# thanosDelatolas/eva-vos

Measured on AMD Instinct MI355X. Metric: frames/sec STCN mask-propagate 480p 1-obj, higher is better.
Workload: dtype f32; 1 GPU; DAVIS-17-val-shaped 480x854 (padded 480x864) single-object STCN propagate: fresh engine, interact(mask,0), T=66 frames/video, mem_freq=5, top_k=50; one video per step per GPU; videos_per_gpu=38, streams_per_gpu=4, key_lookahead=0, clips=8 distinct synthetic clips (one per pooled engine), weights=synthetic recipe seed 0 (no checkpoints offline)

## Files before the change

eva_vos_amd/_lib.py:

```python
from __future__ import annotations

import ctypes as C
import os

import torch

_HERE = os.path.dirname(os.path.abspath(__file__))
LIB_PATH = os.environ.get("STCN_LIB") or os.path.join(_HERE, "libstcn_hip.so")

K_CLASSES = ("conv", "conv_reduce", "memread", "elementwise", "conv_n1", "other", "wino_input", "fusion_conv", "attention")


class WeightDesc(C.Structure):
    _fields_ = [("name", C.c_char_p), ("data", C.c_void_p), ("ndim", C.c_int32), ("shape", C.c_int64 * 4)]


class EngineOpts(C.Structure):
    _fields_ = [(n, C.c_int32) for n in ("lookahead", "decode_batch", "key_batch", "fuse_side")]


class ModelOpts(C.Structure):
    _fields_ = [("top_k", C.c_int32), ("km", C.c_float)]


# ... 22 lines not shown
    "stcn_test_transpose": (_I, [_P, _P, _P, _I, _I, _I, _L, _L, _I]),
    "stcn_engine_create": (_I, [_P, _I, _I, _I, _I, _I, _P, _P, _P, _P, C.POINTER(_P)]),
    "stcn_engine_create_ex": (_I, [_P, _I, _I, _I, _I, _I, _P, _P, _P, _P, C.POINTER(EngineOpts), C.POINTER(_P)]),
    "stcn_engine_get_opts": (_I, [_P, C.POINTER(EngineOpts)]),
    "stcn_engine_destroy": (_I, [_P]),
    "stcn_engine_reset": (_I, [_P]),
    "stcn_engine_clone": (_I, [_P, _P, _P, _P, C.POINTER(_P)]),
    "stcn_interact": (_I, [_P, _P, _I, _I, _I]),
    "stcn_get_stats": (_I, [_P, C.POINTER(Stats)]),
    "stcn_get_flops": (_I, [_P, C.POINTER(_D)]),
    "stcn_last_conv_path": (C.c_char_p, []),
    "stcn_test_conv_trace": (_I, [_I]),
    "stcn_test_conv_trace_get": (C.c_char_p, []),
    "stcn_test_conv": (_I, [_P, _P, _P, _P, _P, _P] + [_I] * 11),
    "stcn_test_conv_ex": (_I, [_P, _P, _P, _P, _P, _P] + [_I] * 11 + [_P, _I, _L, _L, _L, _I, _L]),
    "stcn_test_conv_path": (_I, [_I] * 9 + [C.c_char_p, _I]),
    "stcn_test_conv_plan": (_I, [_I] * 9 + [C.POINTER(C.c_int32), _I, C.POINTER(_D)]),
    "stcn_test_sweep_plan": (_I, [_I, _I, _I, _I, C.POINTER(C.c_int32), _I, C.POINTER(C.c_int32)]),
    "stcn_test_encode_key": (_I, [_P, _P, _P, _I, _I, _P, _P, _P, _P, _P]),
    "stcn_test_encode_value": (_I, [_P, _P, _P, _P, _P, _I, _I, _I, _P]),
    "stcn_test_memory_read": (_I, [_P, _P, _P, _P, _I, _I, _I, _P, _P, _P]),
    "stcn_test_memory_read_k": (_I, [_P, _P, _P, _P, _I, _I, _I, _I, _P, _P, _P]),
    "stcn_test_memory_read_km": (_I, [_P, _P, _P, _P, _I, _I, _I, _I, _I, _I, _F, _P, _P, _P, _P]),
    "stcn_bench_memory_read": (_I, [_P, _P, _P, _P, _I, _I, _I, _I, _P, C.POINTER(_F), C.POINTER(C.c_int32)]),
    "stcn_bench_memory_read_k": (_I, [_P, _P, _P, _P, _I, _I, _I, _I, _I, _P, C.POINTER(_F), C.POINTER(C.c_int32)]),
    "stcn_bench_memory_read_km": (_I, [_P, _P, _P, _P, _I, _I, _I, _I, _I, _I, _F, _I, _P, C.POINTER(_F), C.POINTER(C.c_int32)]),
    "stcn_memread_plan": (_I, [_I, _I, C.POINTER(C.c_int32)]),
    "stcn_memread_scratch": (_I, [_I, C.POINTER(C.c_int64)]),
    "stcn_test_kernel": (_I, [C.c_char_p, _P, C.POINTER(_P), _I, C.POINTER(C.c_int64), _I, C.POINTER(_D), _I]),
    "stcn_test_fail_at": (_I, [_I]),
# ... 63 lines not shown
```

eva_vos_amd/csrc/engine.cpp:

```cpp
#include "engine.h"
#include "src_hash.h"

#include <algorithm>
#include <atomic>
#include <cmath>
#include <cstdarg>
#include <cstdio>
#include <cstdlib>
#include <cstring>
#include <map>
#include <mutex>
#include <unordered_map>
#include <utility>

namespace stcn {

static thread_local char g_err[512] = "";
void set_error(const char *fmt, ...) {
    va_list ap;
    va_start(ap, fmt);
    vsnprintf(g_err, sizeof(g_err), fmt, ap);
    va_end(ap);
}
const char *get_error() { return g_err; }
// ... 480 lines not shown
    p.kn = w.kn;
    pl = ConvPlan{};
    pl.fl = 2.0 * p.M * p.N * (double)(cw.kh * cw.kw * cw.cin);
    if (a.force_splitk <= 0 && (fusion_conv_plan(p, pl) || wino4_plan(p, m.wino4_min_wg, w.wino_v_floats, w.splitk_floats, pl) ||
                                wino_plan(p, w.wino_v_floats, w.splitk_floats, pl)))
        return STCN_OK;
    conv_plan(p, a.force_splitk, w.splitk_floats, pl);
    return STCN_OK;
}

int run_conv(const Model &m, Work &w, hipStream_t s, const std::string &name, const ConvArgs &a) {
    ConvP p;
    ConvPlan &pl = g_path.plan;
    const int rc = plan_conv(m, w, name, a, p, pl);
    if (rc) return rc;
    hipEvent_t *eg[W4_MAX_CHUNKS] = {}, *ei[W4_MAX_CHUNKS] = {}, *er = nullptr;
    if (w.prof) {
        const double in0 = (double)(p.bs0 ? p.B : 1) * p.H * p.W * p.c0, in1 = p.x1 ? (double)(p.bs1 ? p.B : 1) * p.H * p.W * p.c1 : 0.0;
        const double resb = p.res ? (p.res_bs ? (double)p.M * p.N : (double)p.OH * p.OW * p.N) : 0.0;
        const double bytes = 4.0 * (in0 + in1 + (double)p.N * p.K + (double)p.M * p.N + resb);
        const bool hbm_bound = pl.fl / bytes < 157.3e12 / 8.0e12;
        const int cls = w.conv_cls;
        const bool hbm_acc = hbm_bound && cls == STCN_K_CONV;
        w.prof->bytes[cls] += bytes;
        w.prof->flops[cls] += pl.fl;
        w.prof->exec_flops[cls] += pl.fl_exec;
        if (hbm_acc) { w.prof->hbm_conv_bytes += bytes; w.prof->hbm_conv_flops += pl.fl; }
        if (pl.family == CONV_WINO4) w.prof->wino4_flops += pl.fl; else if (pl.family == CONV_WINO2) w.prof->wino2_flops += pl.fl;
        for (int c = 0; c < pl.n_gemm; ++c) {
            eg[c] = w.prof->attach(cls, hbm_acc);
            if (c < pl.n_in) ei[c] = w.prof->attach(STCN_K_WINO_INPUT);
        }
        if (pl.reduce) er = w.prof->attach(STCN_K_CONV_REDUCE);
    }
    if (g_trace_on) { char b[96]; g_trace += name; g_trace += '='; g_trace += format_conv_path(pl, b, sizeof(b)); g_trace += '\n'; }
    switch (pl.family) {
    case CONV_FUSION: fusion_conv_launch(p, pl, s, eg[0]); break;
    case CONV_WINO4: wino4_launch(p, pl, w.wino_v, s, ei, eg, er); break;
    case CONV_WINO2: wino_launch(p, pl, w.wino_v, s, ei[0], eg[0], er); break;
    default: conv_launch(p, s, eg[0], er);
    }
    return launch_status(name.c_str());
}

#define RC(x) do { int rc_ = (x); if (rc_) return rc_; } while (0)

int encode_key(const Model &m, Work &w, hipStream_t s, const float *img4, const KeyOut &o, int B, long out_bs) {
    const Dims &d = w.d;
    const long obs = B > 1 ? out_bs : 0;
    const long ibs = obs ? obs : CONV_DENSE;
    RC(run_conv(m, w, s, "key_encoder.conv1", ConvArgs(img4, 4, B, d.nh, d.nw).strided(2).out(w.A).relu(0, 1)));
    { Scope sc(w.prof, STCN_K_ELEMWISE, s); maxpool3x3s2_launch(w.A, w.B, B, d.h2, d.w2, 64, s); }
    struct St { const char *name; int n, planes, stride; } stages[3] = {{"res2", 3, 64, 1}, {"layer2", 4, 128, 2}, {"layer3", 6, 256, 2}};
// ... 20 lines not shown
            if (o.s4) RC(run_conv(m, w, s, "decoder.up_8_4.skip_conv", ConvArgs(x, 256, B, d.h4, d.w4).out(o.s4, obs)));
        } else if (si == 1) {
            if (o.f8_copy) HIPCHK(hipMemcpyAsync(o.f8_copy, x, (size_t)d.hw8 * 512 * 4, hipMemcpyDeviceToDevice, s));
            if (o.s8) RC(run_conv(m, w, s, "decoder.up_16_8.skip_conv", ConvArgs(x, 512, B, d.h8, d.w8).out(o.s8, obs)));
        }
    }
    if (o.k16) {
        RC(run_conv(m, w, s, "key_proj.key_proj", ConvArgs(o.f16, 1024, B, d.h16, d.w16, ibs).out(o.k16, obs)));
        if (o.msq) {
            Scope sc(w.prof, STCN_K_ELEMWISE, s);
            rowsumsq_launch(o.k16, d.hw16, 64, o.msq, s, B, out_bs, out_bs);
        }
    }
    if (o.f16_thin) RC(run_conv(m, w, s, "key_comp", ConvArgs(o.f16, 1024, B, d.h16, d.w16, ibs).out(o.f16_thin, obs)));
    if (o.f16_thin && o.dthin) {
        RC(run_conv(m, w, s, "decoder.compress.downsample#b", ConvArgs(o.f16_thin, 512, B, d.h16, d.w16, ibs).out(o.dthin, obs)));
        RC(run_conv(m, w, s, "decoder.compress.conv1#b", ConvArgs(o.f16_thin, 512, B, d.h16, d.w16, ibs).out(o.cthin, obs).relu(1, 0)));
    }
    return STCN_OK;
}

int value_frame_parts(const Model &m, Work &w, hipStream_t s, const float *f16, float *vd, float *vc) {
    const Dims &d = w.d;
    RC(run_conv(m, w, s, "value_encoder.fuser.block1.downsample#b", ConvArgs(f16, 1024, 1, d.h16, d.w16).out(vd)));
    RC(run_conv(m, w, s, "value_encoder.fuser.block1.conv1#b", ConvArgs(f16, 1024, 1, d.h16, d.w16).out(vc).relu(1, 0)));
    return STCN_OK;
}

static int resblock_split(const Model &m, Work &w, hipStream_t s, const std::string &p, const float *x, int c, int B,
                          int H, int W, const float *dpart, const float *cpart, long part_bs, int part_bmod, float *t1, float *t2,
                          float *out, long out_bs) {
    const ConvW &cw = m.c(p + ".conv1");
    RC(run_conv(m, w, s, p + ".downsample#a", ConvArgs(x, c, B, H, W).out(t2).residual(dpart, part_bs, part_bmod)));
    RC(run_conv(m, w, s, p + ".conv1#a", ConvArgs(x, c, B, H, W).out(t1).residual(cpart, part_bs, part_bmod).relu(1, 1)));
    RC(run_conv(m, w, s, p + ".conv2", ConvArgs(t1, cw.cout, B, H, W).out(out, out_bs).residual(t2)));
    return STCN_OK;
}

static int resblock(const Model &m, Work &w, hipStream_t s, const std::string &p, const float *x0, int c0, long bs0,
                    const float *x1, int c1, long bs1, int B, int H, int W, float *t1, float *t2, float *out,
                    long out_bs) {
    const ConvW &cw = m.c(p + ".conv1");
    const ConvArgs in = ConvArgs(x0, c0, B, H, W, bs0).concat(x1, c1, bs1);
    const float *skip; long skip_bs;
    if (m.conv.count(p + ".downsample")) {
        RC(run_conv(m, w, s, p + ".downsample", ConvArgs(in).out(t2)));
        skip = t2; skip_bs = CONV_DENSE;
    } else { skip = x0; skip_bs = bs0; }
    RC(run_conv(m, w, s, p + ".conv1", ConvArgs(in).out(t1).relu(1, 1)));
    RC(run_conv(m, w, s, p + ".conv2", ConvArgs(t1, cw.cout, B, H, W).out(out, out_bs).residual(skip, skip_bs)));
    return STCN_OK;
}

int encode_value(const Model &m, Work &w, hipStream_t s, const float *img4, const float *f16, const float *masks,
                 long mask_stride, float *out, long out_bs, const float *vd, const float *vc) {
    const Dims &d = w.d;
    const int k = w.k;
    { Scope sc(w.prof, STCN_K_ELEMWISE, s); pack_value_input_launch(img4, masks, mask_stride, k, (int)d.npix, w.vin, s); }
    RC(run_conv(m, w, s, "value_encoder.conv1", ConvArgs(w.vin, 8, k, d.nh, d.nw).strided(2).out(w.C).relu(0, 1)));
    { Scope sc(w.prof, STCN_K_ELEMWISE, s); maxpool3x3s2_launch(w.C, w.B, k, d.h2, d.w2, 64, s); }
    int H = d.h4, W = d.w4, cin = 64;
    const int planes[3] = {64, 128, 256}, strides[3] = {1, 2, 2};
    for (int li = 0; li < 3; ++li)
        for (int i = 0; i < 2; ++i) {
// ... 859 lines not shown
```

eva_vos_amd/csrc/engine.h:

```cpp
#pragma once
#include <hip/hip_runtime.h>

#include <deque>
#include <map>
#include <memory>
#include <set>
#include <string>
#include <vector>

#include "../../include/stcn_hip.h"
#include "kernels.h"

namespace stcn {

void set_error(const char *fmt, ...);
struct Model;
struct ConvW;
hipError_t pool_malloc(void **p, size_t bytes);
void pool_free(void *p);
void pool_release();
bool wants_wino(const ConvW &cw);
bool wants_wino4(const ConvW &cw);
bool wants_wino_fusion12(const ConvW &cw);
int make_wino(Model &m, ConvW &cw, const std::vector<float> &w_host);
// ... 57 lines not shown
    void end(hipStream_t s);
    int collect(float *ms);
    ~Prof();
private:
    Ev &push_pair(int cls, bool hbm);
};

size_t wino_v_capacity(const Dims &d, int maxb);
struct Work {
    Dims d{};
    int k = 0;
    size_t S = 0;
    float *A = nullptr, *B = nullptr, *C = nullptr, *D = nullptr;
    float *splitk = nullptr; size_t splitk_floats = 0;
    float *wino_v = nullptr; size_t wino_v_floats = 0;
    float *cbam = nullptr;
    float *readout = nullptr;
    float *logit4 = nullptr;
    float *flogit = nullptr;
    float *agg = nullptr;
    float *agg_alt = nullptr;
    float *pooled = nullptr, *amap = nullptr, *attn = nullptr;
    float *cand_v = nullptr; int32_t *cand_i = nullptr, *cand_n = nullptr;
    float *gmax = nullptr, *tau = nullptr;
    int32_t *centre = nullptr;
    float *qk = nullptr;
    float *vin = nullptr;
    Prof *prof = nullptr;
    Knobs kn = Knobs::from_env();
    int conv_cls = STCN_K_CONV;
// ... 6 lines not shown
void inject_failure_after(int n);
int launch_status(const char *what);
const char *last_conv_path();
void set_conv_path(const char *s);
void conv_trace(int on);
const char *conv_trace_get();
constexpr long CONV_DENSE = -1;
struct ConvArgs {
    const float *x0 = nullptr, *x1 = nullptr;
    int c0 = 0, c1 = 0;
    long bs0 = CONV_DENSE, bs1 = 0;
    int B = 1, H = 0, W = 0, stride = 1;
    float *y = nullptr; long y_bs = 0;
    const float *res = nullptr; long res_bs = CONV_DENSE; int res_bmod = 0;
    int relu_in = 0, relu_out = 0, force_splitk = 0;
    ConvArgs(const float *x, int c, int B_, int H_, int W_, long bs = CONV_DENSE) : x0(x), c0(c), bs0(bs), B(B_), H(H_), W(W_) {}
    ConvArgs &concat(const float *x, int c, long bs) { x1 = x; c1 = c; bs1 = bs; return *this; }
    ConvArgs &strided(int s) { stride = s; return *this; }
    ConvArgs &out(float *y_, long bs = 0) { y = y_; y_bs = bs; return *this; }
    ConvArgs &residual(const float *r, long bs = CONV_DENSE, int bmod = 0) { res = r; res_bs = bs; res_bmod = bmod; return *this; }
    ConvArgs &relu(int in, int out_) { relu_in = in; relu_out = out_; return *this; }
    ConvArgs &splitk(int k) { force_splitk = k; return *this; }
};
int plan_conv(const Model &m, const Work &w, const std::string &name, const ConvArgs &a, ConvP &p, ConvPlan &pl);
const char *format_conv_path(const ConvPlan &pl, char *out, size_t n);
int run_conv(const Model &m, Work &w, hipStream_t s, const std::string &name, const ConvArgs &a);
struct SweepGroup {
    int first;
    int t_lo;
    int G;
    bool inserts;
};
std::vector<SweepGroup> plan_sweep(int idx, int closest, int mem_freq, int cap);
constexpr int MAX_DECODE_GROUP = 8;
int encode_key(const Model &m, Work &w, hipStream_t s, const float *img4, const KeyOut &o, int B = 1, long out_bs = 0);
int encode_value(const Model &m, Work &w, hipStream_t s, const float *img4, const float *f16,
                 const float *masks, long mask_stride, float *out, long out_bs, const float *vd = nullptr,
// ... 61 lines not shown
```

eva_vos_amd/csrc/hooks.cpp:

```cpp
#include <algorithm>
#include <climits>
#include <cmath>
#include <cstdlib>
#include <cstring>
#include <string>
#include <vector>

#include "engine.h"

using namespace stcn;
#define RC(x) do { int rc_ = (x); if (rc_) return rc_; } while (0)

namespace {
struct TmpWork {
    Work w;
    int rc;
    TmpWork(int nh, int nw, int k) { rc = w.init(nh, nw, k); }
    ~TmpWork() { (void)hipDeviceSynchronize(); w.release(); }
};
struct DevBuf {
    float *p = nullptr;
    int alloc(size_t floats) { HIPCHK(hipMalloc((void **)&p, floats * 4)); return STCN_OK; }
    ~DevBuf() { if (p) { (void)hipDeviceSynchronize(); (void)hipFree(p); } }
};
// ... 1 lines not shown
    ConvW cw;
    cw.cout = Cout; cw.cin = Cin; cw.cin_p = Cin; cw.kh = KH; cw.kw = KW;
    cw.K = KH * KW * Cin; cw.Kp = (cw.K + 31) / 32 * 32;
    return cw;
}
size_t test_wino_v_floats(int B, int OH, int OW, int Cin) {
    const size_t v2 = (size_t)16 * Cin * (((size_t)B * ((OH + 1) / 2) * ((OW + 1) / 2) + 63) / 64 * 64);
    const size_t v4 = (size_t)36 * Cin * (((size_t)B * ((OH + 3) / 4) * ((OW + 3) / 4) + 127) / 128 * 128);
    return v2 > v4 ? v2 : v4;
}
struct ConvRig {
    Model m;
    Work w;
    DevBuf wv, ws;
    ~ConvRig() { (void)hipDeviceSynchronize(); for (void *p : m.allocs) (void)hipFree(p); }
    int init(ConvW cw, const std::vector<float> *hw, bool f4, int B, int OH, int OW, size_t slab_floats) {
        if (hw) {
            RC(make_wino(m, cw, *hw));
            RC(make_wino_fusion12(m, cw, *hw));
            if (f4) RC(make_wino4(m, cw, *hw));
            w.wino_v_floats = test_wino_v_floats(B, OH, OW, cw.cin_p);
            RC(wv.alloc(w.wino_v_floats));
            w.wino_v = wv.p;
        }
        m.conv["t"] = cw;
        w.splitk_floats = slab_floats;
        RC(ws.alloc(w.splitk_floats));
        w.splitk = ws.p;
        return STCN_OK;
    }
};
int plan_test_conv(int B, int H, int W, int Cin, int Cout, int K, int stride, int flags, int splitk, ConvP &p, ConvPlan &pl) {
    static float buf[4];
    Model m;
    ConvW cw = test_convw(Cin, Cout, K, K);
    cw.w = cw.bias = buf;
// ... 86 lines not shown
        HIPCHK(hipMemcpy(hw.data(), wpad.p, hw.size() * 4, hipMemcpyDeviceToHost));
    }
    ConvRig r;
    RC(r.init(cw, wino ? &hw : nullptr, flags & 4, B, OH, OW, (size_t)16 * 1024 * 1024));
    if (wino && (flags & 4)) r.m.wino4_min_wg = 0;
    if (Cout == 1) {
        const bool dense = !x1 && bs0 == CONV_DENSE && y_bs == CONV_DENSE && !res;
        if (stride != 1 || !dense) { set_error("Cout==1 path is stride 1, one dense source, dense output, no residual"); return STCN_E_INVALID; }
        float b0 = 0.f;
        if (bias) HIPCHK(hipMemcpy(&b0, bias, 4, hipMemcpyDeviceToHost));
        conv_n1_launch(x, wpad.p, b0, y, B, H, W, Cin, KH, flags & 1, s);
        set_conv_path("n1");
    } else {
        RC(run_conv(r.m, r.w, s, "t", ConvArgs(x, Cin, B, H, W, bs0).concat(x1, c1, x1 ? bs1 : 0).strided(stride).out(y, y_bs == CONV_DENSE ? 0 : y_bs)
                                          .residual(res, res_bs, res_bmod).relu(flags & 1, (flags >> 1) & 1).splitk(splitk)));
    }
    HIPCHK(hipStreamSynchronize(s));
    HIPCHK(hipGetLastError());
    return STCN_OK;
}

int stcn_test_conv_path(int B, int H, int W, int Cin, int Cout, int K, int stride, int flags, int splitk, char *out, int n) {
    if (Cin % 4 || !out || n < 1) { set_error("stcn_test_conv_path: Cin%%4==0 and an output buffer required"); return STCN_E_INVALID; }
    ConvP p;
    ConvPlan pl;
    RC(plan_test_conv(B, H, W, Cin, Cout, K, stride, flags, splitk, p, pl));
    format_conv_path(pl, out, (size_t)n);
    return STCN_OK;
}

// ... 401 lines not shown
```

eva_vos_amd/csrc/kernels.h:

```cpp
#pragma once
#include <hip/hip_runtime.h>
#include <stdint.h>

#include <cstdlib>

#include "../../include/stcn_hip.h"

namespace stcn {

struct FastDiv {
    unsigned magic, shift, d;
};
static inline FastDiv fastdiv_make(unsigned d) {
    FastDiv f{0, 0, d};
    if (d <= 1) return f;
    unsigned s = 0;
    while ((1ull << s) < d) ++s;
    f.magic = (unsigned)(((1ull << (31 + s)) / d) + 1);
    f.shift = s - 1;
    return f;
}
#if defined(__HIPCC__)
__device__ __forceinline__ int fastdiv(int x, const FastDiv f) {
    return f.d <= 1 ? x : (int)(__umulhi((unsigned)x, f.magic) >> f.shift);
// ... 72 lines not shown
    double fl = 0;
    double fl_exec = 0;
};
void conv_plan(ConvP &p, int force_splitk, size_t workspace_floats, ConvPlan &pl);
void conv_launch(const ConvP &p, hipStream_t s, hipEvent_t *ev_gemm = nullptr, hipEvent_t *ev_red = nullptr);
void conv_reduce_launch(const ConvP &p, hipStream_t s, hipEvent_t *ev_red = nullptr);
bool wino_plan(const ConvP &p, size_t v_cap, size_t slab_floats, ConvPlan &pl);
void wino_launch(const ConvP &p, const ConvPlan &pl, float *V, hipStream_t s, hipEvent_t *ev_in = nullptr, hipEvent_t *ev_gemm = nullptr,
                 hipEvent_t *ev_red = nullptr);
void wino_transform_weights(const float *w, int N, int Cin, int Kp, float *U);
#ifndef W4_MIN_CIN
#define W4_MIN_CIN 64
#endif
bool wino4_plan(const ConvP &p, int min_wg, size_t v_cap, size_t slab_floats, ConvPlan &pl);
void wino4_launch(const ConvP &p, const ConvPlan &pl, float *V, hipStream_t s, hipEvent_t *const *ev_in = nullptr,
                  hipEvent_t *const *ev_gemm = nullptr, hipEvent_t *ev_red = nullptr);
void wino4_transform_weights(const float *w, int N, int Cin, int Kp, float *U);
bool wino_enabled();
int wino4_mode();

bool fusion_conv_plan(const ConvP &p, ConvPlan &pl);
void fusion_conv_launch(const ConvP &p, const ConvPlan &pl, hipStream_t s, hipEvent_t *ev_gemm = nullptr);

void conv_n1_launch(const float *x, const float *w, float bias, float *y, int B, int H, int W, int C,
                    int KH, int relu_in, hipStream_t s);

void maxpool3x3s2_launch(const float *x, float *y, int B, int H, int W, int C, hipStream_t s);
void pack_image_launch(const float *img_chw, float *out, int H, int W, int nh, int nw, int lw, int lh,
                       hipStream_t s);
void pack_value_input_launch(const float *img4, const float *masks, long mask_stride, int k, int npix,
                             float *out, hipStream_t s);
// ... 81 lines not shown
```

eva_vos_amd/csrc/winograd4.hip:

```cpp
#include <hip/hip_ext.h>

#include <cstdio>
#include <cstdlib>
#include <type_traits>

#include "wino_common.h"

namespace stcn {

typedef float f32x4 __attribute__((ext_vector_type(4)));
typedef float f32x16 __attribute__((ext_vector_type(16)));

#ifdef STCN_W4_CLOCK
__device__ unsigned long long g_w4_clock[2 * 8192];
#if STCN_W4_CLOCK == 2
#define W4_MFMA(a_, b_, c_) w4_fake_mfma(a_, b_, c_)
#endif
#endif
#ifndef W4_MFMA
#define W4_MFMA(a_, b_, c_) __builtin_amdgcn_mfma_f32_32x32x2f32(a_, b_, c_, 0, 0, 0)
#endif

static constexpr int W4T = 32;
static constexpr int W4N = 32;
// ... 7 lines not shown
}
#endif

__device__ __forceinline__ void bt6(const f32x4 &d0, const f32x4 &d1, const f32x4 &d2, const f32x4 &d3, const f32x4 &d4, const f32x4 &d5,
                                    f32x4 &o0, f32x4 &o1, f32x4 &o2, f32x4 &o3, f32x4 &o4, f32x4 &o5) {
    o0 = d0 * 1.265625f - d2 * 2.8125f + d4;
    const f32x4 e1 = d4 - d2 * 2.25f, f1 = d3 * 0.75f - d1 * 1.6875f;
    o1 = e1 + f1;
    o2 = e1 - f1;
    const f32x4 e2 = d4 - d2 * 0.5625f, f2 = d3 * 1.5f - d1 * 0.84375f;
    o3 = e2 + f2;
    o4 = e2 - f2;
    o5 = d1 * 1.265625f - d3 * 2.8125f + d5;
}

__global__ __launch_bounds__(256) void wino4_input_kernel(const float *__restrict__ x, unsigned x_bytes, long x_bs, int H, int W, int C,
                                                          int relu_in, int TH, int TW, int Mt, int Mt_pad, int cb_per_chunk,
                                                          int tile_lo, int tile_hi, float *__restrict__ V) {
    const long i = xcd_contiguous_block((int)blockIdx.x, (int)gridDim.x) * 256L + threadIdx.x;
    const int c16 = (int)(i & 7);
    const long tile = tile_lo + (i >> 3);
    if (tile >= tile_hi) return;
    const int KB = C / 8, NCB = C / 32;
    const int cb0 = blockIdx.y * cb_per_chunk, cb1 = min(NCB, cb0 + cb_per_chunk);
    const bool live = tile < Mt;
    const int tpi = TH * TW;
    const int b = live ? (int)(tile / tpi) : 0;
    const int r = live ? (int)(tile - (long)b * tpi) : 0;
    const int ty = r / TW, tx = r - ty * TW;
    const int y0 = 4 * ty - 1, x0 = 4 * tx - 1;
    unsigned long long ok = 0;
#pragma unroll
    for (int yy = 0; yy < 6; ++yy)
#pragma unroll
        for (int xx = 0; xx < 6; ++xx)
            if (live && (unsigned)(y0 + yy) < (unsigned)H && (unsigned)(x0 + xx) < (unsigned)W) ok |= 1ull << (yy * 6 + xx);
    const __amdgpu_buffer_rsrc_t rx = __builtin_amdgcn_make_buffer_rsrc(const_cast<float *>(x), 0, x_bytes, 0x00020000);
    const int xoff = (int)((b * x_bs + ((long)y0 * W + x0) * C + 4 * c16) * 4);
    const long ps = ((long)KB * Mt_pad) << 3;
    const float lo = relu_in ? 0.f : -__builtin_inff();
    for (int cb = cb0; cb < cb1; ++cb) {
        f32x4 t[6][6];
#pragma unroll
        for (int xx = 0; xx < 6; ++xx) {
            f32x4 d[6];
#pragma unroll
            for (int yy = 0; yy < 6; ++yy) {
                const unsigned vo = ((ok >> (yy * 6 + xx)) & 1ull) ? (unsigned)(xoff + ((yy * W + xx) * C + 32 * cb) * 4) : 0x80000000u;
                f32x4 v = __builtin_bit_cast(f32x4, __builtin_amdgcn_raw_buffer_load_b128(rx, vo, 0, 0));
                v.x = fmaxf(v.x, lo); v.y = fmaxf(v.y, lo); v.z = fmaxf(v.z, lo); v.w = fmaxf(v.w, lo);
                d[yy] = v;
            }
            bt6(d[0], d[1], d[2], d[3], d[4], d[5], t[0][xx], t[1][xx], t[2][xx], t[3][xx], t[4][xx], t[5][xx]);
        }
        const int kb = cb * 4 + (c16 >> 1);
        float *base = V + (((long)kb * Mt_pad + tile) << 3) + 4 * (c16 & 1);
#pragma unroll
        for (int xi = 0; xi < 6; ++xi) {
            f32x4 v[6];
            bt6(t[xi][0], t[xi][1], t[xi][2], t[xi][3], t[xi][4], t[xi][5], v[0], v[1], v[2], v[3], v[4], v[5]);
            float *dst = base + (long)(xi * 6) * ps;
#pragma unroll
            for (int nu = 0; nu < 6; ++nu) *reinterpret_cast<f32x4 *>(dst + nu * ps) = v[nu];
        }
    }
}

struct Wino4G {
    const float *V, *U;
    unsigned v_bytes, u_bytes;
    int Mt, Mt_pad, KB, N;
    int TH, TW, OH, OW, B, M;
    const float *bias, *res;
    long res_bs; int res_bmod;
    float *y; long y_bs;
    int relu_out;
    FastDiv fd_tpi, fd_tw, fd_tiles_n;
    int full_wg, pieces, kb_per_piece;
    float *partial;
    int tm0;
// ... 359 lines not shown
    const WinoGeom ge = wino_geom(p, 4, 2 * W4T);
    if (!wino_extents_ok(p, 36, ge.Mt_pad)) return false;
    const W4Plan w4 = wino4_gemm_plan(p, ge, slab_floats);
    if (wino4_mode() < 2 && w4.judge_wg < min_wg) return false;
    const size_t need = (size_t)36 * p.Cin * ge.Mt_pad;
    if (need > v_cap) return false;
    cp.family = CONV_WINO4;
    cp.geo = ge; cp.w4 = w4;
    cp.v_floats = need;
    cp.n_in = cp.n_gemm = w4.chunks; cp.reduce = w4.pieces > 1;
    cp.fl_exec = 2.0 * (double)need * p.N;
    return true;
}

void wino4_launch(const ConvP &p, const ConvPlan &cp, float *V, hipStream_t s, hipEvent_t *const *ev_in, hipEvent_t *const *ev_gemm,
                  hipEvent_t *ev_red) {
    const W4Plan &pl = cp.w4;
    const WinoGeom &ge = cp.geo;
    const int tiles_n = pl.tiles_n, mb = pl.mb, tiles_m = pl.tiles_m;
    Wino4G g{};
    wino_fill_desc(g, p, ge, 36, V, p.wino4_u, tiles_n);
    g.full_wg = pl.full_wg; g.pieces = pl.pieces; g.kb_per_piece = pl.per; g.partial = p.partial;
    g.xb_m = g.xb_n = g.xb_cols = 0;
    {
        const int rows = pl.full_wg / tiles_n;
        if (pl.chunks == 1 && pl.full_wg % 8 == 0 && rows * tiles_n == pl.full_wg && tiles_n >= 8) {
            const int per = pl.full_wg / 8;
            int best = 0, best_sum = per % tiles_n == 0 ? per / tiles_n + tiles_n : rows + tiles_n;
            for (int bn = 2; bn <= tiles_n; ++bn) {
                if (per % bn || tiles_n % bn) continue;
                const int bm = per / bn;
                if (bm < 1 || rows % bm || (rows / bm) * (tiles_n / bn) != 8) continue;
                if (bm + bn < best_sum) { best_sum = bm + bn; best = bn; }
            }
            if (best && best != tiles_n) { g.xb_n = best; g.xb_m = per / best; g.xb_cols = tiles_n / best; }
        }
    }
    const size_t lds = (size_t)36 * W4T * W4N * sizeof(float);
    for (int c = 0; c < pl.chunks; ++c) {
        const int tm_lo = c * pl.tm_per_chunk, tm_hi = tm_lo + pl.tm_per_chunk < tiles_m ? tm_lo + pl.tm_per_chunk : tiles_m;
        const int tile_lo = tm_lo * W4T * mb, tile_hi = pl.chunks == 1 ? ge.Mt_pad : tm_hi * W4T * mb;
        hipEvent_t *ei = ev_in ? ev_in[c] : nullptr, *eg = ev_gemm ? ev_gemm[c] : nullptr;
        const WinoInGrid ig = wino_input_grid(tile_hi - tile_lo, p.Cin);
        launch(wino4_input_kernel, dim3(ig.gx, ig.chunks), dim3(256), 0, s, ei, p.x0, p.x0_bytes, p.bs0, p.H, p.W, p.Cin, p.relu_in, ge.TH, ge.TW,
               ge.Mt, ge.Mt_pad, ig.per, tile_lo, tile_hi, V);
        g.tm0 = tm_lo;
        if (mb == 2) {
            const int grid = (tm_hi - tm_lo) * tiles_n;
            launch(wino4_gemm_kernel<2>, dim3(grid), dim3(64 * W4W), lds, s, eg, g, tiles_n);
        } else {
            launch(wino4_gemm_kernel<1>, dim3(pl.grid), dim3(64 * W4W), lds, s, eg, g, tiles_n);
            if (g.pieces > 1) launch(wino4_reduce_kernel, dim3((tiles_m * tiles_n - g.full_wg) * 64), dim3(256), 0, s, ev_red, g, tiles_n);
        }
    }
}

void wino4_transform_weights(const float *w, int N, int Cin, int Kp, float *U) {
    static const double G[6][3] = {{64.0 / 81, 0, 0},
                                   {-128.0 / 243, -32.0 / 81, -8.0 / 27},
                                   {-128.0 / 243, 32.0 / 81, -8.0 / 27},
// ... 14 lines not shown
```

include/stcn_hip.h:

```cpp
#ifndef STCN_HIP_H
#define STCN_HIP_H

#include <stddef.h>
#include <stdint.h>

#ifdef __cplusplus
extern "C" {
#endif

#define STCN_OK            0
#define STCN_E_INVALID    -1
#define STCN_E_MISSING    -2
#define STCN_E_HIP        -3
#define STCN_E_STATE      -4

#define STCN_MAX_OBJECTS  32

typedef struct stcn_model  stcn_model;
typedef struct stcn_engine stcn_engine;

typedef struct {
    const char  *name;
    const float *data;
    int32_t      ndim;
// ... 53 lines not shown
int stcn_stage_attention(stcn_stage *s, const float *mk16, const float *pos, const float *neg, const float *qk16, int b, float *attn);
int stcn_stage_fusion(stcn_stage *s, const float *im, const float *seg1, const float *seg2, const float *attn, float nc, float nr, float *logit);
int stcn_aggregate_wbg(void *stream, const float *prob, int k, long npix, int keep_bg, int hard, float *out);
int stcn_fusion_model_create(int device, const stcn_weight_desc *fuse, int n_fuse, stcn_model **out);
int stcn_test_transpose(void *stream, const float *src, float *dst, int B, int R, int C, long ld, long planes_bs, int to_rows);


int stcn_test_conv(void *stream, const float *x, const float *w, const float *bias, const float *res,
                   float *y, int B, int H, int W, int Cin, int Cout, int KH, int KW, int stride,
                   int pad, int flags, int splitk);

int stcn_test_conv_ex(void *stream, const float *x, const float *w, const float *bias, const float *res,
                      float *y, int B, int H, int W, int Cin, int Cout, int KH, int KW, int stride,
                      int pad, int flags, int splitk, const float *x1, int c1, long bs0, long bs1, long res_bs, int res_bmod, long y_bs);

int stcn_test_conv_path(int B, int H, int W, int Cin, int Cout, int K, int stride, int flags, int splitk, char *out, int n);
#define STCN_CONV_PLAN_INTS 27
int stcn_test_conv_plan(int B, int H, int W, int Cin, int Cout, int K, int stride, int flags, int splitk, int32_t *iv, int n, double *dv);
const char *stcn_last_conv_path(void);
int stcn_test_sweep_plan(int idx, int closest, int mem_freq, int cap, int32_t *out, int n, int32_t *count);
int stcn_test_conv_trace(int on);
const char *stcn_test_conv_trace_get(void);

int stcn_test_kernel(const char *name, void *stream, void *const *ptrs, int nptr, const int64_t *iv, int ni, const double *fv, int nf);

int stcn_test_encode_key(const stcn_model *m, void *stream, const float *img, int nh, int nw,
                         float *k16, float *f16_thin, float *f16, float *f8, float *f4);

int stcn_test_encode_value(const stcn_model *m, void *stream, const float *img, const float *f16,
                           const float *masks, int k, int nh, int nw, float *out);
// ... 71 lines not shown
```

Measured before the change: 822.5 frames/s.

## Reuse Winograd F4 input transform across sibling convs and restructure input kernel via LDS

Adds tagging of the Winograd F(4x4) transformed input buffer so a conv that reads the same input as the previous one (downsample/conv1 pairs) skips its input transform, optionally producing a second ReLU'd copy in the same pass (dual mode). The input transform kernel is rewritten to have each thread load one column, do the row transform, exchange through LDS, and finish the column transform, which cuts redundant loads of overlapping tiles. This removes repeated input-transform launches and global reads, at the cost of extra workspace for the dual copy, extra LDS barriers, and tag-validity bookkeeping that could go stale if buffers change.

Measured after the change: 826.3 frames/s, median of 5. About the same (+0.5%).

```diff
diff --git a/eva_vos_amd/_lib.py b/eva_vos_amd/_lib.py
--- a/eva_vos_amd/_lib.py
+++ b/eva_vos_amd/_lib.py
@@ -60,6 +60,9 @@
     "stcn_test_conv_trace_get": (C.c_char_p, []),
     "stcn_test_conv": (_I, [_P, _P, _P, _P, _P, _P] + [_I] * 11),
     "stcn_test_conv_ex": (_I, [_P, _P, _P, _P, _P, _P] + [_I] * 11 + [_P, _I, _L, _L, _L, _I, _L]),
+    "stcn_test_conv_pair": (_I, [_P] * 6 + [_I] * 8 + [C.POINTER(C.c_int32)]),
+    "stcn_test_wino4_input": (_I, [_P, _P] + [_I] * 6 + [_P, _P]),
+    "stcn_bench_wino4_input": (_I, [_P, _P] + [_I] * 7 + [_P, _P, C.POINTER(_F)]),
     "stcn_test_conv_path": (_I, [_I] * 9 + [C.c_char_p, _I]),
     "stcn_test_conv_plan": (_I, [_I] * 9 + [C.POINTER(C.c_int32), _I, C.POINTER(_D)]),
     "stcn_test_sweep_plan": (_I, [_I, _I, _I, _I, C.POINTER(C.c_int32), _I, C.POINTER(C.c_int32)]),
diff --git a/eva_vos_amd/csrc/engine.cpp b/eva_vos_amd/csrc/engine.cpp
--- a/eva_vos_amd/csrc/engine.cpp
+++ b/eva_vos_amd/csrc/engine.cpp
@@ -518,6 +518,29 @@
     ConvPlan &pl = g_path.plan;
     const int rc = plan_conv(m, w, name, a, p, pl);
     if (rc) return rc;
+    Work::VTag prev[2] = {w.v_tag[0], w.v_tag[1]};
+    const int n_prev = w.n_v_tag;
+    w.n_v_tag = 0;
+    const bool f4_whole = pl.family == CONV_WINO4 && pl.w4.chunks == 1;
+    const Work::VTag *have = nullptr;
+    float *v2 = nullptr;
+    if (f4_whole && a.v_reuse)
+        for (int i = 0; i < n_prev && !have; ++i) {
+            const Work::VTag &t = prev[i];
+            if (t.x == p.x0 && t.bs0 == p.bs0 && t.B == p.B && t.H == p.H && t.W == p.W && t.C == p.Cin && (t.relu == p.relu_in || a.v_nonneg) &&
+                t.off + pl.v_floats <= w.wino_v_floats)
+                have = &t;
+        }
+    if (have) {
+        pl.n_in = 0;
+        w.v_tag[0] = prev[0]; w.v_tag[1] = prev[1]; w.n_v_tag = n_prev;
+        ++w.v_reused;
+    } else if (pl.family == CONV_WINO4) {
+        if (f4_whole && a.v_dual && !p.relu_in && 2 * pl.v_floats <= w.wino_v_floats) v2 = w.wino_v + pl.v_floats;
+        w.v_tag[0] = Work::VTag{p.x0, p.bs0, p.B, p.H, p.W, p.Cin, p.relu_in, 0};
+        w.n_v_tag = 1;
+        if (v2) { w.v_tag[1] = w.v_tag[0]; w.v_tag[1].relu = 1; w.v_tag[1].off = pl.v_floats; w.n_v_tag = 2; }
+    }
     hipEvent_t *eg[W4_MAX_CHUNKS] = {}, *ei[W4_MAX_CHUNKS] = {}, *er = nullptr;
     if (w.prof) {
         const double in0 = (double)(p.bs0 ? p.B : 1) * p.H * p.W * p.c0, in1 = p.x1 ? (double)(p.bs1 ? p.B : 1) * p.H * p.W * p.c1 : 0.0;
@@ -540,7 +563,7 @@
     if (g_trace_on) { char b[96]; g_trace += name; g_trace += '='; g_trace += format_conv_path(pl, b, sizeof(b)); g_trace += '\n'; }
     switch (pl.family) {
     case CONV_FUSION: fusion_conv_launch(p, pl, s, eg[0]); break;
-    case CONV_WINO4: wino4_launch(p, pl, w.wino_v, s, ei, eg, er); break;
+    case CONV_WINO4: wino4_launch(p, pl, w.wino_v + (have ? have->off : 0), s, ei, eg, er, have != nullptr, v2); break;
     case CONV_WINO2: wino_launch(p, pl, w.wino_v, s, ei[0], eg[0], er); break;
     default: conv_launch(p, s, eg[0], er);
     }
@@ -591,8 +614,8 @@
     }
     if (o.f16_thin) RC(run_conv(m, w, s, "key_comp", ConvArgs(o.f16, 1024, B, d.h16, d.w16, ibs).out(o.f16_thin, obs)));
     if (o.f16_thin && o.dthin) {
-        RC(run_conv(m, w, s, "decoder.compress.downsample#b", ConvArgs(o.f16_thin, 512, B, d.h16, d.w16, ibs).out(o.dthin, obs)));
-        RC(run_conv(m, w, s, "decoder.compress.conv1#b", ConvArgs(o.f16_thin, 512, B, d.h16, d.w16, ibs).out(o.cthin, obs).relu(1, 0)));
+        RC(run_conv(m, w, s, "decoder.compress.downsample#b", ConvArgs(o.f16_thin, 512, B, d.h16, d.w16, ibs).out(o.dthin, obs).dual_v()));
+        RC(run_conv(m, w, s, "decoder.compress.conv1#b", ConvArgs(o.f16_thin, 512, B, d.h16, d.w16, ibs).out(o.cthin, obs).relu(1, 0).reuse_v()));
     }
     return STCN_OK;
 }
@@ -600,7 +623,7 @@
 int value_frame_parts(const Model &m, Work &w, hipStream_t s, const float *f16, float *vd, float *vc) {
     const Dims &d = w.d;
     RC(run_conv(m, w, s, "value_encoder.fuser.block1.downsample#b", ConvArgs(f16, 1024, 1, d.h16, d.w16).out(vd)));
-    RC(run_conv(m, w, s, "value_encoder.fuser.block1.conv1#b", ConvArgs(f16, 1024, 1, d.h16, d.w16).out(vc).relu(1, 0)));
+    RC(run_conv(m, w, s, "value_encoder.fuser.block1.conv1#b", ConvArgs(f16, 1024, 1, d.h16, d.w16).out(vc).relu(1, 0).reuse_v(true)));
     return STCN_OK;
 }
 
@@ -608,8 +631,8 @@
                           int H, int W, const float *dpart, const float *cpart, long part_bs, int part_bmod, float *t1, float *t2,
                           float *out, long out_bs) {
     const ConvW &cw = m.c(p + ".conv1");
-    RC(run_conv(m, w, s, p + ".downsample#a", ConvArgs(x, c, B, H, W).out(t2).residual(dpart, part_bs, part_bmod)));
-    RC(run_conv(m, w, s, p + ".conv1#a", ConvArgs(x, c, B, H, W).out(t1).residual(cpart, part_bs, part_bmod).relu(1, 1)));
+    RC(run_conv(m, w, s, p + ".downsample#a", ConvArgs(x, c, B, H, W).out(t2).residual(dpart, part_bs, part_bmod).dual_v()));
+    RC(run_conv(m, w, s, p + ".conv1#a", ConvArgs(x, c, B, H, W).out(t1).residual(cpart, part_bs, part_bmod).relu(1, 1).reuse_v()));
     RC(run_conv(m, w, s, p + ".conv2", ConvArgs(t1, cw.cout, B, H, W).out(out, out_bs).residual(t2)));
     return STCN_OK;
 }
@@ -620,11 +643,14 @@
     const ConvW &cw = m.c(p + ".conv1");
     const ConvArgs in = ConvArgs(x0, c0, B, H, W, bs0).concat(x1, c1, bs1);
     const float *skip; long skip_bs;
-    if (m.conv.count(p + ".downsample")) {
-        RC(run_conv(m, w, s, p + ".downsample", ConvArgs(in).out(t2)));
+    const bool has_ds = m.conv.count(p + ".downsample") != 0;
+    if (has_ds) {
+        RC(run_conv(m, w, s, p + ".downsample", ConvArgs(in).out(t2).dual_v()));
         skip = t2; skip_bs = CONV_DENSE;
     } else { skip = x0; skip_bs = bs0; }
-    RC(run_conv(m, w, s, p + ".conv1", ConvArgs(in).out(t1).relu(1, 1)));
+    ConvArgs a1 = ConvArgs(in).out(t1).relu(1, 1);
+    if (has_ds) a1.reuse_v();
+    RC(run_conv(m, w, s, p + ".conv1", a1));
     RC(run_conv(m, w, s, p + ".conv2", ConvArgs(t1, cw.cout, B, H, W).out(out, out_bs).residual(skip, skip_bs)));
     return STCN_OK;
 }
diff --git a/eva_vos_amd/csrc/engine.h b/eva_vos_amd/csrc/engine.h
--- a/eva_vos_amd/csrc/engine.h
+++ b/eva_vos_amd/csrc/engine.h
@@ -95,6 +95,9 @@
     float *A = nullptr, *B = nullptr, *C = nullptr, *D = nullptr;
     float *splitk = nullptr; size_t splitk_floats = 0;
     float *wino_v = nullptr; size_t wino_v_floats = 0;
+    struct VTag { const float *x = nullptr; long bs0 = 0; int B = 0, H = 0, W = 0, C = 0, relu = 0; size_t off = 0; };
+    VTag v_tag[2]; int n_v_tag = 0;
+    int v_reused = 0;
     float *cbam = nullptr;
     float *readout = nullptr;
     float *logit4 = nullptr;
@@ -131,6 +134,7 @@
     float *y = nullptr; long y_bs = 0;
     const float *res = nullptr; long res_bs = CONV_DENSE; int res_bmod = 0;
     int relu_in = 0, relu_out = 0, force_splitk = 0;
+    bool v_dual = false, v_reuse = false, v_nonneg = false;
     ConvArgs(const float *x, int c, int B_, int H_, int W_, long bs = CONV_DENSE) : x0(x), c0(c), bs0(bs), B(B_), H(H_), W(W_) {}
     ConvArgs &concat(const float *x, int c, long bs) { x1 = x; c1 = c; bs1 = bs; return *this; }
     ConvArgs &strided(int s) { stride = s; return *this; }
@@ -138,6 +142,8 @@
     ConvArgs &residual(const float *r, long bs = CONV_DENSE, int bmod = 0) { res = r; res_bs = bs; res_bmod = bmod; return *this; }
     ConvArgs &relu(int in, int out_) { relu_in = in; relu_out = out_; return *this; }
     ConvArgs &splitk(int k) { force_splitk = k; return *this; }
+    ConvArgs &dual_v() { v_dual = true; return *this; }
+    ConvArgs &reuse_v(bool nonneg = false) { v_reuse = true; v_nonneg = nonneg; return *this; }
 };
 int plan_conv(const Model &m, const Work &w, const std::string &name, const ConvArgs &a, ConvP &p, ConvPlan &pl);
 const char *format_conv_path(const ConvPlan &pl, char *out, size_t n);
diff --git a/eva_vos_amd/csrc/hooks.cpp b/eva_vos_amd/csrc/hooks.cpp
--- a/eva_vos_amd/csrc/hooks.cpp
+++ b/eva_vos_amd/csrc/hooks.cpp
@@ -7,6 +7,7 @@
 #include <vector>
 
 #include "engine.h"
+#include "wino_common.h"
 
 using namespace stcn;
 #define RC(x) do { int rc_ = (x); if (rc_) return rc_; } while (0)
@@ -39,12 +40,12 @@
     Work w;
     DevBuf wv, ws;
     ~ConvRig() { (void)hipDeviceSynchronize(); for (void *p : m.allocs) (void)hipFree(p); }
-    int init(ConvW cw, const std::vector<float> *hw, bool f4, int B, int OH, int OW, size_t slab_floats) {
+    int init(ConvW cw, const std::vector<float> *hw, bool f4, int B, int OH, int OW, size_t slab_floats, int v_copies = 1) {
         if (hw) {
             RC(make_wino(m, cw, *hw));
             RC(make_wino_fusion12(m, cw, *hw));
             if (f4) RC(make_wino4(m, cw, *hw));
-            w.wino_v_floats = test_wino_v_floats(B, OH, OW, cw.cin_p);
+            w.wino_v_floats = test_wino_v_floats(B, OH, OW, cw.cin_p) * v_copies;
             RC(wv.alloc(w.wino_v_floats));
             w.wino_v = wv.p;
         }
@@ -161,6 +162,83 @@
     } else {
         RC(run_conv(r.m, r.w, s, "t", ConvArgs(x, Cin, B, H, W, bs0).concat(x1, c1, x1 ? bs1 : 0).strided(stride).out(y, y_bs == CONV_DENSE ? 0 : y_bs)
                                           .residual(res, res_bs, res_bmod).relu(flags & 1, (flags >> 1) & 1).splitk(splitk)));
+    }
+    HIPCHK(hipStreamSynchronize(s));
+    HIPCHK(hipGetLastError());
+    return STCN_OK;
+}
+
+int stcn_test_conv_pair(void *stream, const float *x, const float *wgt, const float *bias, float *y1, float *y2, int B, int H, int W, int Cin,
+                        int Cout, int flags1, int flags2, int mode, int32_t *reused) {
+    if (!x || !wgt || !y1 || !y2 || !reused || B < 1 || H < 1 || W < 1 || Cin < 4 || Cin % 4 || Cout < 2) {
+        set_error("stcn_test_conv_pair: x, w, y1, y2, reused, B, H, W >= 1, Cin%%4==0, Cout >= 2 required"); return STCN_E_INVALID;
+    }
+    hipStream_t s = (hipStream_t)stream;
+    ConvW cw = test_convw(Cin, Cout, 3, 3);
+    DevBuf wpad;
+    RC(wpad.alloc((size_t)Cout * cw.Kp));
+    HIPCHK(hipMemsetAsync(wpad.p, 0, (size_t)Cout * cw.Kp * 4, s));
+    HIPCHK(hipMemcpy2DAsync(wpad.p, (size_t)cw.Kp * 4, wgt, (size_t)cw.K * 4, (size_t)cw.K * 4, Cout, hipMemcpyDeviceToDevice, s));
+    cw.w = wpad.p; cw.bias = const_cast<float *>(bias);
+    HIPCHK(hipStreamSynchronize(s));
+    std::vector<float> hw((size_t)Cout * cw.Kp);
+    HIPCHK(hipMemcpy(hw.data(), wpad.p, hw.size() * 4, hipMemcpyDeviceToHost));
+    ConvRig r;
+    RC(r.init(cw, &hw, true, B, H, W, (size_t)16 * 1024 * 1024, (mode & 16) ? 1 : 2));
+    r.m.wino4_min_wg = 0;
+    auto args = [&](float *y, int flags) { return ConvArgs(x, Cin, B, H, W).out(y).relu(flags & 1, (flags >> 1) & 1); };
+    ConvArgs a1 = args(y1, flags1), a2 = args(y2, flags2);
+    if (mode & 1) a1.dual_v();
+    if (mode & 2) a2.reuse_v((mode & 4) != 0);
+    if (mode & 16) {
+        ConvP p;
+        ConvPlan pl;
+        RC(plan_conv(r.m, r.w, "t", a1, p, pl));
+        if (pl.v_floats) r.w.wino_v_floats = pl.v_floats;
+    }
+    RC(run_conv(r.m, r.w, s, "t", a1));
+    if (mode & 8) RC(run_conv(r.m, r.w, s, "t", args(y2, flags1 ^ 1)));
+    RC(run_conv(r.m, r.w, s, "t", a2));
+    *reused = r.w.v_reused;
+    HIPCHK(hipStreamSynchronize(s));
+    HIPCHK(hipGetLastError());
+    return STCN_OK;
+}
+
+int stcn_test_wino4_input(void *stream, const float *x, int B, int H, int W, int C, int relu, int chunk_mb, float *V_out, float *V2_out) {
+    return stcn_bench_wino4_input(stream, x, B, H, W, C, relu, chunk_mb, 0, V_out, V2_out, nullptr);
+}
+
+int stcn_bench_wino4_input(void *stream, const float *x, int B, int H, int W, int C, int relu, int chunk_mb, int iters, float *V_out, float *V2_out,
+                           float *ms) {
+    if (!x || !V_out || B < 1 || H < 1 || W < 1 || C < 32 || C % 32 || chunk_mb < 0 || (V2_out && relu) || iters < 0 || (iters > 0 && !ms)) {
+        set_error("stcn_test_wino4_input: x and V_out, B, H, W >= 1, C a multiple of 32, chunk_mb >= 0 required; the dual form takes relu = 0; timed runs need ms");
+        return STCN_E_INVALID;
+    }
+    ConvP p{};
+    p.x0 = x; p.c0 = p.Cin = C; p.B = B; p.H = p.OH = H; p.W = p.OW = W; p.bs0 = (long)H * W * C; p.relu_in = relu != 0; p.N = 32;
+    const WinoGeom ge = wino_geom(p, 4, 64);
+    const long xb = (long)B * p.bs0 * 4, vb = 36L * C * ge.Mt_pad * 4;
+    if (xb >= (1L << 31) || vb >= (1L << 32)) { set_error("stcn_test_wino4_input: x of %ld bytes or V of %ld bytes beyond what the kernel addresses", xb, vb); return STCN_E_INVALID; }
+    p.x0_bytes = (unsigned)xb;
+    long n = chunk_mb > 0 ? (vb + ((long)chunk_mb << 20) - 1) / ((long)chunk_mb << 20) : 1;
+    n = n > W4_MAX_CHUNKS ? W4_MAX_CHUNKS : n;
+    const int wt = ge.Mt_pad / 64, per = (int)((wt + n - 1) / n) * 64;
+    hipStream_t s = (hipStream_t)stream;
+    auto run = [&]() { for (int lo = 0; lo < ge.Mt_pad; lo += per) wino4_input_launch(p, ge, lo, lo + per < ge.Mt_pad ? lo + per : ge.Mt_pad, V_out, V2_out, s); };
+    if (iters > 0) {
+        hipEvent_t e0, e1;
+        HIPCHK(hipEventCreate(&e0)); HIPCHK(hipEventCreate(&e1));
+        run(); run();
+        HIPCHK(hipEventRecord(e0, s));
+        for (int i = 0; i < iters; ++i) run();
+        HIPCHK(hipEventRecord(e1, s));
+        HIPCHK(hipEventSynchronize(e1));
+        HIPCHK(hipEventElapsedTime(ms, e0, e1));
+        *ms /= (float)iters;
+        (void)hipEventDestroy(e0); (void)hipEventDestroy(e1);
+    } else {
+        run();
     }
     HIPCHK(hipStreamSynchronize(s));
     HIPCHK(hipGetLastError());
diff --git a/eva_vos_amd/csrc/kernels.h b/eva_vos_amd/csrc/kernels.h
--- a/eva_vos_amd/csrc/kernels.h
+++ b/eva_vos_amd/csrc/kernels.h
@@ -110,7 +110,8 @@
 #endif
 bool wino4_plan(const ConvP &p, int min_wg, size_t v_cap, size_t slab_floats, ConvPlan &pl);
 void wino4_launch(const ConvP &p, const ConvPlan &pl, float *V, hipStream_t s, hipEvent_t *const *ev_in = nullptr,
-                  hipEvent_t *const *ev_gemm = nullptr, hipEvent_t *ev_red = nullptr);
+                  hipEvent_t *const *ev_gemm = nullptr, hipEvent_t *ev_red = nullptr, bool v_ready = false, float *V2 = nullptr);
+void wino4_input_launch(const ConvP &p, const WinoGeom &ge, int tile_lo, int tile_hi, float *V, float *V2, hipStream_t s, hipEvent_t *ev = nullptr);
 void wino4_transform_weights(const float *w, int N, int Cin, int Kp, float *U);
 bool wino_enabled();
 int wino4_mode();
diff --git a/eva_vos_amd/csrc/winograd4.hip b/eva_vos_amd/csrc/winograd4.hip
--- a/eva_vos_amd/csrc/winograd4.hip
+++ b/eva_vos_amd/csrc/winograd4.hip
@@ -45,56 +45,120 @@
     o5 = d1 * 1.265625f - d3 * 2.8125f + d5;
 }
 
-__global__ __launch_bounds__(256) void wino4_input_kernel(const float *__restrict__ x, unsigned x_bytes, long x_bs, int H, int W, int C,
-                                                          int relu_in, int TH, int TW, int Mt, int Mt_pad, int cb_per_chunk,
-                                                          int tile_lo, int tile_hi, float *__restrict__ V) {
-    const long i = xcd_contiguous_block((int)blockIdx.x, (int)gridDim.x) * 256L + threadIdx.x;
-    const int c16 = (int)(i & 7);
-    const long tile = tile_lo + (i >> 3);
-    if (tile >= tile_hi) return;
+static constexpr int W4I_S = 8;
+static constexpr int W4I_THREADS = 384;
+static constexpr int W4I_COL = 9;
+static constexpr int W4I_START = 320;
+static constexpr int W4I_START_TILE = 20;
+static constexpr int W4I_SPARE = W4I_START + W4I_S * W4I_START_TILE;
+static constexpr int W4I_ROW = 496;
+
+__device__ __forceinline__ void w4i_lds_barrier() {
+    __builtin_amdgcn_fence(__ATOMIC_RELEASE, "workgroup", "local");
+    __builtin_amdgcn_s_barrier();
+    __builtin_amdgcn_fence(__ATOMIC_ACQUIRE, "workgroup", "local");
+}
+
+template <bool DUAL>
+__global__ __launch_bounds__(W4I_THREADS) void wino4_input_kernel(const float *__restrict__ x, unsigned x_bytes, long x_bs, int H, int W, int C,
+                                                                  int relu_in, int TH, int TW, int Mt, int Mt_pad, int cb_per_chunk,
+                                                                  int tile_lo, int tile_hi, float *__restrict__ V, float *__restrict__ V2) {
+    __shared__ f32x4 lds[6 * W4I_ROW];
+    const long t0 = tile_lo + (long)xcd_contiguous_block((int)blockIdx.x, (int)gridDim.x) * W4I_S;
+    const int tid = threadIdx.x;
     const int KB = C / 8, NCB = C / 32;
     const int cb0 = blockIdx.y * cb_per_chunk, cb1 = min(NCB, cb0 + cb_per_chunk);
-    const bool live = tile < Mt;
     const int tpi = TH * TW;
-    const int b = live ? (int)(tile / tpi) : 0;
-    const int r = live ? (int)(tile - (long)b * tpi) : 0;
-    const int ty = r / TW, tx = r - ty * TW;
-    const int y0 = 4 * ty - 1, x0 = 4 * tx - 1;
-    unsigned long long ok = 0;
+    struct Tile { bool live, start; int b, y0, x0; };
+    auto tile_of = [&](int s) {
+        const long tile = t0 + s;
+        Tile t;
+        t.live = tile < Mt;
+        t.b = t.live ? (int)(tile / tpi) : 0;
+        const int r = t.live ? (int)(tile - (long)t.b * tpi) : 0;
+        const int ty = r / TW, tx = r - ty * TW;
+        t.y0 = 4 * ty - 1; t.x0 = 4 * tx - 1;
+        t.start = s == 0 || tx == 0;
+        return t;
+    };
+    const bool main_col = tid < 256;
+    const int c16a = tid & 7;
+    const int sa = main_col ? tid >> 5 : (tid - 256) >> 4;
+    const int ka = main_col ? ((tid >> 3) & 3) + 2 : ((tid - 256) >> 3) & 1;
+    const Tile ta = tile_of(sa);
+    const bool write_a = main_col || ta.start;
+    const bool load_a = ta.live && write_a && (unsigned)(ta.x0 + ka) < (unsigned)W;
+    unsigned ok = 0;
 #pragma unroll
     for (int yy = 0; yy < 6; ++yy)
-#pragma unroll
-        for (int xx = 0; xx < 6; ++xx)
-            if (live && (unsigned)(y0 + yy) < (unsigned)H && (unsigned)(x0 + xx) < (unsigned)W) ok |= 1ull << (yy * 6 + xx);
+        if (load_a && (unsigned)(ta.y0 + yy) < (unsigned)H) ok |= 1u << yy;
     const __amdgpu_buffer_rsrc_t rx = __builtin_amdgcn_make_buffer_rsrc(const_cast<float *>(x), 0, x_bytes, 0x00020000);
-    const int xoff = (int)((b * x_bs + ((long)y0 * W + x0) * C + 4 * c16) * 4);
+    const int xoff = (int)((ta.b * x_bs + ((long)ta.y0 * W + ta.x0 + ka) * C + 4 * c16a) * 4);
+    const int slot_a = main_col ? (4 * sa + ka) * W4I_COL + c16a
+                                : (ta.start ? W4I_START + sa * W4I_START_TILE + ka * W4I_COL + c16a : W4I_SPARE + (c16a & 3));
+    const int xi = tid >> 6, lane = tid & 63;
+    const int half = lane & 1, sb = (lane >> 1) & 7, kbq = lane >> 4;
+    const Tile tb = tile_of(sb);
+    const long tile_b = t0 + sb;
+    const int main_b = xi * W4I_ROW + 4 * sb * W4I_COL + 2 * kbq + half;
+    const int slot_b01 = tb.start ? xi * W4I_ROW + W4I_START + sb * W4I_START_TILE + 2 * kbq + half : main_b;
     const long ps = ((long)KB * Mt_pad) << 3;
-    const float lo = relu_in ? 0.f : -__builtin_inff();
+    const float lo = DUAL || !relu_in ? -__builtin_inff() : 0.f;
     for (int cb = cb0; cb < cb1; ++cb) {
-        f32x4 t[6][6];
-#pragma unroll
-        for (int xx = 0; xx < 6; ++xx) {
-            f32x4 d[6];
-#pragma unroll
-            for (int yy = 0; yy < 6; ++yy) {
-                const unsigned vo = ((ok >> (yy * 6 + xx)) & 1ull) ? (unsigned)(xoff + ((yy * W + xx) * C + 32 * cb) * 4) : 0x80000000u;
-                f32x4 v = __builtin_bit_cast(f32x4, __builtin_amdgcn_raw_buffer_load_b128(rx, vo, 0, 0));
-                v.x = fmaxf(v.x, lo); v.y = fmaxf(v.y, lo); v.z = fmaxf(v.z, lo); v.w = fmaxf(v.w, lo);
-                d[yy] = v;
+        f32x4 d[6];
+#pragma unroll
+        for (int yy = 0; yy < 6; ++yy) {
+            const unsigned vo = ((ok >> yy) & 1u) ? (unsigned)(xoff + (yy * W * C + 32 * cb) * 4) : 0x80000000u;
+            d[yy] = __builtin_bit_cast(f32x4, __builtin_amdgcn_raw_buffer_load_b128(rx, vo, 0, 0));
+        }
+#pragma unroll
+        for (int phase = 0; phase < (DUAL ? 2 : 1); ++phase) {
+            const float l = phase ? 0.f : lo;
+            float *Vp = phase ? V2 : V;
+            f32x4 t[6];
+            {
+                f32x4 e[6];
+#pragma unroll
+                for (int yy = 0; yy < 6; ++yy) {
+                    const f32x4 v = d[yy];
+                    e[yy].x = fmaxf(v.x, l); e[yy].y = fmaxf(v.y, l); e[yy].z = fmaxf(v.z, l); e[yy].w = fmaxf(v.w, l);
+                }
+                bt6(e[0], e[1], e[2], e[3], e[4], e[5], t[0], t[1], t[2], t[3], t[4], t[5]);
             }
-            bt6(d[0], d[1], d[2], d[3], d[4], d[5], t[0][xx], t[1][xx], t[2][xx], t[3][xx], t[4][xx], t[5][xx]);
-        }
-        const int kb = cb * 4 + (c16 >> 1);
-        float *base = V + (((long)kb * Mt_pad + tile) << 3) + 4 * (c16 & 1);
-#pragma unroll
-        for (int xi = 0; xi < 6; ++xi) {
+#pragma unroll
+            for (int row = 0; row < 6; ++row) lds[row * W4I_ROW + slot_a] = t[row];
+            w4i_lds_barrier();
+#pragma unroll
+            for (int k = 0; k < 6; ++k) t[k] = lds[(k < 2 ? slot_b01 : main_b) + k * W4I_COL];
             f32x4 v[6];
-            bt6(t[xi][0], t[xi][1], t[xi][2], t[xi][3], t[xi][4], t[xi][5], v[0], v[1], v[2], v[3], v[4], v[5]);
-            float *dst = base + (long)(xi * 6) * ps;
-#pragma unroll
-            for (int nu = 0; nu < 6; ++nu) *reinterpret_cast<f32x4 *>(dst + nu * ps) = v[nu];
-        }
-    }
+            bt6(t[0], t[1], t[2], t[3], t[4], t[5], v[0], v[1], v[2], v[3], v[4], v[5]);
+            if (tile_b < tile_hi) {
+                float *dst = Vp + (((long)(cb * 4 + kbq) * Mt_pad + tile_b) << 3) + 4 * half + (long)(xi * 6) * ps;
+#pragma unroll
+                for (int nu = 0; nu < 6; ++nu) *reinterpret_cast<f32x4 *>(dst + nu * ps) = v[nu];
+            }
+            w4i_lds_barrier();
+        }
+    }
+}
+
+static WinoInGrid wino4_input_grid(long tiles, int Cin) {
+    const unsigned gx = (unsigned)((tiles + W4I_S - 1) / W4I_S);
+    const int NCB = Cin / 32;
+    int chunks = (int)((2048 + gx - 1) / gx);
+    chunks = chunks < 1 ? 1 : (chunks > NCB ? NCB : chunks);
+    const int per = (NCB + chunks - 1) / chunks;
+    return {gx, (NCB + per - 1) / per, per};
+}
+
+void wino4_input_launch(const ConvP &p, const WinoGeom &ge, int tile_lo, int tile_hi, float *V, float *V2, hipStream_t s, hipEvent_t *ev) {
+    const WinoInGrid ig = wino4_input_grid(tile_hi - tile_lo, p.Cin);
+    if (V2)
+        launch(wino4_input_kernel<true>, dim3(ig.gx, ig.chunks), dim3(W4I_THREADS), 0, s, ev, p.x0, p.x0_bytes, p.bs0, p.H, p.W, p.Cin, 0, ge.TH, ge.TW,
+               ge.Mt, ge.Mt_pad, ig.per, tile_lo, tile_hi, V, V2);
+    else
+        launch(wino4_input_kernel<false>, dim3(ig.gx, ig.chunks), dim3(W4I_THREADS), 0, s, ev, p.x0, p.x0_bytes, p.bs0, p.H, p.W, p.Cin, p.relu_in, ge.TH,
+               ge.TW, ge.Mt, ge.Mt_pad, ig.per, tile_lo, tile_hi, V, V2);
 }
 
 struct Wino4G {
@@ -484,7 +548,7 @@
 }
 
 void wino4_launch(const ConvP &p, const ConvPlan &cp, float *V, hipStream_t s, hipEvent_t *const *ev_in, hipEvent_t *const *ev_gemm,
-                  hipEvent_t *ev_red) {
+                  hipEvent_t *ev_red, bool v_ready, float *V2) {
     const W4Plan &pl = cp.w4;
     const WinoGeom &ge = cp.geo;
     const int tiles_n = pl.tiles_n, mb = pl.mb, tiles_m = pl.tiles_m;
@@ -511,9 +575,7 @@
         const int tm_lo = c * pl.tm_per_chunk, tm_hi = tm_lo + pl.tm_per_chunk < tiles_m ? tm_lo + pl.tm_per_chunk : tiles_m;
         const int tile_lo = tm_lo * W4T * mb, tile_hi = pl.chunks == 1 ? ge.Mt_pad : tm_hi * W4T * mb;
         hipEvent_t *ei = ev_in ? ev_in[c] : nullptr, *eg = ev_gemm ? ev_gemm[c] : nullptr;
-        const WinoInGrid ig = wino_input_grid(tile_hi - tile_lo, p.Cin);
-        launch(wino4_input_kernel, dim3(ig.gx, ig.chunks), dim3(256), 0, s, ei, p.x0, p.x0_bytes, p.bs0, p.H, p.W, p.Cin, p.relu_in, ge.TH, ge.TW,
-               ge.Mt, ge.Mt_pad, ig.per, tile_lo, tile_hi, V);
+        if (!v_ready) wino4_input_launch(p, ge, tile_lo, tile_hi, V, V2, s, ei);
         g.tm0 = tm_lo;
         if (mb == 2) {
             const int grid = (tm_hi - tm_lo) * tiles_n;
diff --git a/include/stcn_hip.h b/include/stcn_hip.h
--- a/include/stcn_hip.h
+++ b/include/stcn_hip.h
@@ -91,6 +91,12 @@
                       float *y, int B, int H, int W, int Cin, int Cout, int KH, int KW, int stride,
                       int pad, int flags, int splitk, const float *x1, int c1, long bs0, long bs1, long res_bs, int res_bmod, long y_bs);
 
+int stcn_test_conv_pair(void *stream, const float *x, const float *w, const float *bias, float *y1, float *y2, int B, int H, int W, int Cin,
+                        int Cout, int flags1, int flags2, int mode, int32_t *reused);
+int stcn_test_wino4_input(void *stream, const float *x, int B, int H, int W, int C, int relu, int chunk_mb, float *V_out, float *V2_out);
+int stcn_bench_wino4_input(void *stream, const float *x, int B, int H, int W, int C, int relu, int chunk_mb, int iters, float *V_out, float *V2_out,
+                           float *ms);
+
 int stcn_test_conv_path(int B, int H, int W, int Cin, int Cout, int K, int stride, int flags, int splitk, char *out, int n);
 #define STCN_CONV_PLAN_INTS 27
 int stcn_test_conv_plan(int B, int H, int W, int Cin, int Cout, int K, int stride, int flags, int splitk, int32_t *iv, int n, double *dv);
```
